# HumanCompatibleAI/imitation

Hardware: AMD Instinct MI355X
Metric: env-steps/sec (gen+disc round) GAIL HalfCheetah n_envs=1024 (higher is better)
Workload: dtype f32

## Files before the change

imitation_amd/csrc/policy.hip:

```cpp
#include "common.h"
#include "rn_common.h"
#include <algorithm>
#include <type_traits>
#include <cstring>

#include "../../include/imitation_hip.h"
#include "policy_common.h"

namespace {


template <int H>
struct Lds {
  static constexpr int XS = MAXD + 1, HS = H + 1, AS = MAXA + 1;
  static constexpr int x = 0;
  static constexpr int a1 = x + ROWS * XS;
  static constexpr int a2 = a1 + ROWS * HS;
  static constexpr int dz = a2 + ROWS * HS;
  static constexpr int out = dz + ROWS * HS;
  static constexpr int dout = out + ROWS * AS;
  static constexpr int aux = dout + ROWS * AS;
  static constexpr int total = aux + ROWS * AS + 64;
};

// ... 1443 lines not shown
            dst = b0 + cc * rows + r;
          }
        };
        tr(o.pW1, H, D); tr(o.pW2, H, H); tr(o.vW1, H, D); tr(o.vW2, H, H);
        Pt[dst] = pn;
      }
    }
  }
  if (next_batch > 0 && !stats_block) {
    __syncthreads();
    prepare_stats(d, obs, adv, next_idx, next_batch, T, n_envs, update_norm, nm, nv, ncount, w.advstat, lds);
  }
}

struct CLds {
  static constexpr int RS = 68;
  static constexpr int x = 0;
  static constexpr int a1 = x + MAXD * RS;
  static constexpr int a2 = a1 + 2 * 32 * RS;
  static constexpr int dz2 = a2 + 2 * 32 * RS;
  static constexpr int dz1 = dz2 + 2 * 32 * RS;
  static constexpr int dout = dz1 + 2 * 32 * RS;
  static constexpr int aux = dout + MAXA * RS;
  static constexpr int misc = aux + MAXA * RS;
  static constexpr int scratch = misc + 8 * RS;
  static constexpr int total = scratch + 64;
};


#ifndef IA_UPD_TSTR
#define IA_UPD_TSTR 36
#endif
constexpr int UPD_TSTR = IA_UPD_TSTR;
__host__ __device__ inline int upd_tbase(int off) { return (off * UPD_TSTR + 31) >> 5; }
__host__ __device__ inline int upd_pt4(int P4) { return (upd_tbase(P4) + 3) & ~3; }

template <bool SMALL>
__device__ __forceinline__ void chain_stage_rows(const ia_policy_desc& d, const float* __restrict__ nm,
                                                 const float* __restrict__ nv, const int i0, const int row_lim,
                                                 float* __restrict__ lds, const float* __restrict__ stg, const int tw,
                                                 const int q, const int lane) {
  using L = CLds;
  const int D = d.obs_dim;
  const int S1 = (D + 3) >> 2;
#ifndef IA_SMALL_STAGE_ASIDE
#define IA_SMALL_STAGE_ASIDE 1
#endif
  constexpr int QS = (SMALL && IA_SMALL_STAGE_ASIDE) ? 1 : 0;
  const bool idle = SMALL && q != QS;
  if (!idle) {
    const int rbase = SMALL ? 0 : q * 16;
    const int l128 = lane + 64 * tw;
    const int s1r = (65536 + S1 - 1) / S1;
    for (int g = l128; g < 16 * S1; g += 128) {
      const int r = (g * s1r) >> 16, k0 = (g - r * S1) * 4;
      const bool rok = (i0 + rbase + r) < row_lim;
      float raw[4], mu[4], vr[4];
      {
        const f32x4 rq = *reinterpret_cast<const f32x4*>(stg + UpdStage::x + (rbase * S1 + g) * 4);
        const f32x4 mq = *reinterpret_cast<const f32x4*>(nm + k0);
        const f32x4 vq = *reinterpret_cast<const f32x4*>(nv + k0);
#pragma unroll
        for (int j = 0; j < 4; ++j) {
          raw[j] = rq[j];
          mu[j] = mq[j];
          vr[j] = vq[j];
// ... 30 lines not shown
  const float* __restrict__ stg = stg_in + opaque_zero;
  float* __restrict__ slab = LOCAL ? stg_in + opaque_zero + UpdStage::x : slab_g;
  unsigned long long* __restrict__ slab64 = reinterpret_cast<unsigned long long*>(slab_g);
  auto put = [&](float* p, float v) {
    if constexpr (LOCAL) *p = v;
    else if (ll_xcd) ll_store_xcd(slab64 + (p - slab), v, ll_seq);
    else ll_store_agent(slab64 + (p - slab), v, ll_seq);
  };
  const int batch = rows.batch;
  constexpr int H = 32;
  using L = CLds;
#define IA_TS(slot) do { if (tstamp && i0_in == 0 && threadIdx.x == 0) tstamp[slot] = clock64(); } while (0)
  const int tid = threadIdx.x + opaque_zero, lane = tid & 63;
  const int wv = __builtin_amdgcn_readfirstlane(tid >> 6);
  const int tw = TSPLIT ? split_tw : (SMALL ? (wv & 1) : (wv >> 2)), q = SMALL ? (wv >> 1) : (wv & 3);
  const bool helper = TSPLIT && wv >= 4;
  const int li = lane & 15, lk = lane >> 4;
  const int D = d.obs_dim, A = d.act_dim;
  const PolOff o = pol_offsets(D, A, H, d.discrete);
  const int i0 = i0_in;
  const int aw = d.discrete ? 1 : A;
  const float invB = 1.f / (float)batch;
  const int S1 = (D + 3) >> 2;
  const int oW1 = tw ? o.vW1 : o.pW1, ob1 = tw ? o.vb1 : o.pb1, oW2 = tw ? o.vW2 : o.pW2, ob2 = tw ? o.vb2 : o.pb2;
  const float* __restrict__ sP = sP_in + opaque_zero;
  const float* __restrict__ sPt = sP + ((o.total + 3) & ~3);
  constexpr int TS_ = UPD_TSTR;
  const int tW1 = upd_tbase(oW1), tW2 = upd_tbase(oW2);
  IA_TS(0);

  const int lrow = q * 16 + (lane & 15);
  const bool valid = (i0 + lrow) < row_lim;
  float r_oldlp = 0.f, r_adv = 0.f, r_ret = 0.f, r_act[4] = {0.f, 0.f, 0.f, 0.f};
  constexpr bool HANDOVER = SMALL;
  if (helper) {
  } else if (tw == 0) {
    r_oldlp = stg[UpdStage::oldlp + lrow];
    if constexpr (!HANDOVER) r_adv = stg[UpdStage::adv + lrow];
#pragma unroll
    for (int j = 0; j < 4; ++j) r_act[j] = stg[UpdStage::act + lrow * aw + min(4 * (lane >> 4) + j, aw - 1)];
  } else {
    r_ret = stg[UpdStage::ret + lrow];
    if constexpr (HANDOVER) r_adv = stg[UpdStage::adv + lrow];
  }
  float* gconst = lds + L::scratch + 32;

  IA_TS(9);
  const bool idle = (SMALL && q > 0) || helper;
  if constexpr (!STAGED) chain_stage_rows<SMALL>(d, nm, nv, i0, row_lim, lds, stg, tw, q, lane);
  IA_TS(10);
  constexpr int KT1 = KS1 / 4;
  float fW1[KT1][2][4], fW2[2][2][4], fW2T[2][2][4], fHead[2][4], fHeadT[2][4], b1c[2][4], b2c[2][4], hb[4];
  const int head_base = tw == 0 ? o.aW + min(li, A - 1) * H : o.cW;
  float c_ivar[4] = {1.f, 1.f, 1.f, 1.f}, c_logsd[4] = {0.f, 0.f, 0.f, 0.f};
  if (!helper) {
#pragma unroll
  for (int kt = 0; kt < KT1; ++kt) {
    if (4 * kt < S1) {
#pragma unroll
      for (int t = 0; t < 2; ++t)
#pragma unroll
        for (int r = 0; r < 4; ++r) fW1[kt][t][r] = sPt[tW1 + min(16 * kt + 4 * lk + r, D - 1) * TS_ + 16 * t + li];
    } else {
#pragma unroll
      for (int t = 0; t < 2; ++t)
#pragma unroll
        for (int r = 0; r < 4; ++r) fW1[kt][t][r] = 0.f;
    }
  }
#pragma unroll
  for (int t = 0; t < 2; ++t)
#pragma unroll
    for (int r = 0; r < 4; ++r) b1c[t][r] = sP[ob1 + 16 * t + 4 * lk + r];
  float my_sd = sP[o.log_std + min(lane, A - 1)];
  __builtin_amdgcn_sched_barrier(0);
#pragma unroll
  for (int kt = 0; kt < KT1; ++kt)
#pragma unroll
    for (int t = 0; t < 2; ++t)
#pragma unroll
      for (int r = 0; r < 4; ++r) fW1[kt][t][r] = (16 * kt + 4 * lk + r < D) ? fW1[kt][t][r] : 0.f;
  if constexpr (HANDOVER) {
    if (tw != 0) {
      if (!idle) {
        float advn = r_adv;
        if (normalize_adv && batch > 1) advn = (advn - adv_mean) / (adv_std + 1e-8f);
        if (lk == 0) stg_in[opaque_zero + UpdStage::adv + lrow] = advn;
      }
      if (q == 0 && !d.discrete) {
        const float sd = expf(my_sd);
        const float my_ivar = lane < A ? 1.f / (sd * sd) : 1.f;
        const float my_logsd = lane < A ? logf(sd) : 0.f;
        if (lane < 16) {
          gconst[lane] = my_ivar;
          gconst[16 + lane] = my_logsd;
        }
      }
    }
  } else {
    float my_ivar = 1.f, my_logsd = 0.f;
    if (tw == 0 && !d.discrete) {
      const float sd = expf(my_sd);
      my_ivar = lane < A ? 1.f / (sd * sd) : 1.f;
      my_logsd = lane < A ? logf(sd) : 0.f;
    }
#pragma unroll
    for (int j = 0; j < 4; ++j) {
      c_ivar[j] = __shfl(my_ivar, 4 * lk + j, 64);
      c_logsd[j] = __shfl(my_logsd, 4 * lk + j, 64);
    }
  }
  }
  IA_TS(11);
  __syncthreads();
  IA_TS(1);

  float* a1t = lds + L::a1 + tw * 32 * L::RS;
  float* a2t = lds + L::a2 + tw * 32 * L::RS;
  float* dz2t = lds + L::dz2 + tw * 32 * L::RS;
  float* dz1t = lds + L::dz1 + tw * 32 * L::RS;
  const int trow = 4 * lk * L::RS + q * 16 + li;
  auto xchg16 = [](float v, float& a, float& b) {
    const auto p2 = __builtin_amdgcn_permlane16_swap(__float_as_uint(v), __float_as_uint(v), false, false);
    a = __uint_as_float(p2[0]);
    b = __uint_as_float(p2[1]);
  };
  auto xchg32 = [](float v, float& a, float& b) {
    const auto p2 = __builtin_amdgcn_permlane32_swap(__float_as_uint(v), __float_as_uint(v), false, false);
    a = __uint_as_float(p2[0]);
    b = __uint_as_float(p2[1]);
  };
  auto group_sum = [&](float v) {
    float a, b;
    xchg16(v, a, b);
    v = a + b;
    xchg32(v, a, b);
    return a + b;
  };
  auto group_max = [&](float v) {
    float a, b;
    xchg16(v, a, b);
    v = fmaxf(a, b);
    xchg32(v, a, b);
    return fmaxf(a, b);
  };
  if (!idle) {
  f32x4 a1[2], a2[2];
  {
    f32x4 acc[2][2] = {{{b1c[0][0], b1c[0][1], b1c[0][2], b1c[0][3]}, {0.f, 0.f, 0.f, 0.f}},
                       {{b1c[1][0], b1c[1][1], b1c[1][2], b1c[1][3]}, {0.f, 0.f, 0.f, 0.f}}};
    float xb[KT1][4];
#pragma unroll
    for (int kt = 0; kt < KT1; ++kt)
#pragma unroll
      for (int r = 0; r < 4; ++r) xb[kt][r] = lds[L::x + min(16 * kt + 4 * lk + r, MAXD - 1) * L::RS + q * 16 + li];
    if (HANDOVER && tw == 0) {
      r_adv = stg_in[opaque_zero + UpdStage::adv + lrow];
#pragma unroll
      for (int j = 0; j < 4; ++j) {
        c_ivar[j] = gconst[4 * lk + j];
        c_logsd[j] = gconst[16 + 4 * lk + j];
      }
    }
    __builtin_amdgcn_sched_barrier(0);
#pragma unroll
    for (int kt = 0; kt < KT1; ++kt)
      if (4 * kt < S1) {
#pragma unroll
        for (int r = 0; r < 4; ++r) {
          acc[0][kt & 1] = mfma16(fW1[kt][0][r], xb[kt][r], acc[0][kt & 1]);
          acc[1][kt & 1] = mfma16(fW1[kt][1][r], xb[kt][r], acc[1][kt & 1]);
        }
      }
#pragma unroll
    for (int kt = 0; kt < 2; ++kt)
#pragma unroll
      for (int r = 0; r < 4; ++r)
#pragma unroll
        for (int t = 0; t < 2; ++t) fW2[kt][t][r] = sPt[tW2 + (16 * kt + 4 * lk + r) * TS_ + 16 * t + li];
#pragma unroll
    for (int t = 0; t < 2; ++t)
#pragma unroll
      for (int r = 0; r < 4; ++r) b2c[t][r] = sP[ob2 + 16 * t + 4 * lk + r];
#pragma unroll
    for (int t = 0; t < 2; ++t)
#pragma unroll
      for (int r = 0; r < 4; ++r) {
        a1[t][r] = fast_tanh(acc[t][0][r] + acc[t][1][r]);
        a1t[trow + (16 * t + r) * L::RS] = a1[t][r];
// ... 71 lines not shown
          const float diff = r_act[j] - hout[j];
          logp += -(diff * diff) * (0.5f * c_ivar[j]) - c_logsd[j] - LOG_SQRT_2PI;
          entropy += 0.5f + LOG_SQRT_2PI + c_logsd[j];
        }
      logp = group_sum(logp);
      entropy = group_sum(entropy);
    } else {
      float mx = -3.0e38f, o_act = 0.f;
#pragma unroll
      for (int j = 0; j < 4; ++j)
        if (4 * lk + j < A) {
          mx = fmaxf(mx, hout[j]);
          o_act += (4 * lk + j == act_i) ? hout[j] : 0.f;
        }
      mx = group_max(mx);
      o_act = group_sum(o_act);
      float se = 0.f;
#pragma unroll
      for (int j = 0; j < 4; ++j)
        if (4 * lk + j < A) se += expf(hout[j] - mx);
      lse = mx + logf(group_sum(se));
      logp = o_act - lse;
#pragma unroll
      for (int j = 0; j < 4; ++j)
        if (4 * lk + j < A) {
          const float l = hout[j] - lse;
          entropy -= expf(l) * l;
        }
      entropy = group_sum(entropy);
    }
    IA_TS(13);
    float advn = r_adv;
    if constexpr (!HANDOVER)
      if (normalize_adv && batch > 1) advn = (advn - adv_mean) / (adv_std + 1e-8f);
    const float log_ratio = logp - r_oldlp;
    const float ratio = expf(log_ratio);
    const float lo = 1.f - clip, hi = 1.f + clip;
    const float pl1 = advn * ratio;
    const float pl2 = advn * fminf(fmaxf(ratio, lo), hi);
    const float g1 = pl1 < pl2 ? 1.f : (pl1 == pl2 ? 0.5f : 0.f);
    const float g2 = pl2 < pl1 ? 1.f : (pl1 == pl2 ? 0.5f : 0.f);
    const float inrange = (ratio >= lo && ratio <= hi) ? 1.f : 0.f;
    const float dlogp = valid ? -invB * advn * (g1 + g2 * inrange) * ratio : 0.f;
    IA_TS(14);
    float* doutrow = lds + L::dout + lrow;
    float* auxrow = lds + L::aux + lrow;
    if (!d.discrete) {
#pragma unroll
      for (int j = 0; j < 4; ++j)
        if (4 * lk + j < A) {
          const float diff = r_act[j] - hout[j];
          dout[j] = dlogp * diff * c_ivar[j];
          doutrow[(4 * lk + j) * L::RS] = dout[j];
          auxrow[(4 * lk + j) * L::RS] = valid ? dlogp * (diff * diff * c_ivar[j] - 1.f) - ent_coef * invB : 0.f;
        }
    } else {
#pragma unroll
      for (int j = 0; j < 4; ++j)
        if (4 * lk + j < A) {
          const float l = hout[j] - lse, p = expf(l);
          const float dH = -p * (l + entropy);
          float g = dlogp * ((4 * lk + j == act_i ? 1.f : 0.f) - p);
          g += valid ? -ent_coef * invB * dH : 0.f;
          dout[j] = g;
          doutrow[(4 * lk + j) * L::RS] = g;
        }
    }
// ... 2175 lines not shown
        stats[(long long)mb * 8 + kk] = sv;
        s_st[kk] = sv;
      }
      __syncthreads();
      if (tid == 0) {
        stats[(long long)mb * 8 + 5] = s_st[0] + ent_coef * s_st[2] + vf_coef * s_st[1];
        stats[(long long)mb * 8 + 6] = total_norm;
        stats[(long long)mb * 8 + 7] = coef;
      }
    }
    EP_TS(4);
  }
  tid = threadIdx.x;
#pragma unroll
  for (int j = 0; j < NPC; ++j) {
    const int i = bid * chunk + tid + j * NT;
    if (i < min(o.total, (bid + 1) * chunk)) {
      m[i] = m_[j];
      v[i] = v_[j];
      P[i] = p_[j];
      int dst = i;
      auto tr = [&](int b0, int rows_, int cols) {
        if (i >= b0 && i < b0 + rows_ * cols) {
          const int r = (i - b0) / cols, cc = (i - b0) % cols;
          dst = b0 + cc * rows_ + r;
        }
      };
      tr(o.pW1, H, D); tr(o.pW2, H, H); tr(o.vW1, H, D); tr(o.vW2, H, H);
      Pt[dst] = p_[j];
    }
  }
#undef EP_TS
}

template <int NPT, bool TIMING, int KS1, bool LOCAL, bool SHARD, bool SMALL, bool TSPLIT>
__device__ __forceinline__ void ppo_update_body(
    const ia_policy_desc& d, float* __restrict__ P, float* __restrict__ Pt, float* __restrict__ m, float* __restrict__ v,
    float* __restrict__ nm, float* __restrict__ nv, int32_t* __restrict__ ncount, int update_norm,
    const float* __restrict__ obs, const float* __restrict__ actions, const float* __restrict__ old_logp,
    const float* __restrict__ adv, const float* __restrict__ ret, const int64_t* __restrict__ perm, int T, int n_envs,
    int normalize_adv, float clip, float ent_coef, float vf_coef, float max_norm, float beta1, float beta2, float eps,
    float* __restrict__ ws, int nblk, int n_slices, float* __restrict__ stats, UpdSched sch, int xcd_pack,
    long long* __restrict__ tstamp ,
    ShardArgs sh) {
  constexpr int H = 32;
  using L = CLds;
  extern __shared__ float lds_raw[];
  float* lds = lds_raw + (((16u - (__builtin_amdgcn_groupstaticsize() & 15u)) & 15u) >> 2);
  __shared__ int s_ok, s_pub, s_fail, s_pubw[4];
  if (!TIMING) tstamp = nullptr;
  long long tacc[12] = {0, 0, 0, 0, 0, 0, 0, 0, 0, 0, 0, 0};
  long long tprev = 0;
#define UPD_TS(k) do { if (tstamp && tid == 0) { const long long tn = wall_clock64(); tacc[k] += tn - tprev; tprev = tn; } } while (0)
  if (xcd_pack && (blockIdx.x & 7)) return;
  const int vb = xcd_pack ? blockIdx.x >> 3 : blockIdx.x;
  static_assert(!TSPLIT || (!LOCAL && !SHARD && !SMALL), "one tower per workgroup: several gradient workgroups, one process");
  const int ngw = TSPLIT ? 2 * nblk : nblk;
  const int rb = TSPLIT ? vb >> 1 : vb;
  const int split_tw = TSPLIT ? (vb & 1) : 0;
  const int tid = threadIdx.x;
  const int D = d.obs_dim;
  const PolOff o = pol_offsets(D, d.act_dim, H, d.discrete);
  const UpdWs w = upd_ws(ws, nblk, o.total);
  unsigned* arrivals = w.ctrl + 64;
  unsigned* published = w.ctrl + 1;
  unsigned* sliced = w.ctrl + 16;
// ... 217 lines not shown
    const int jj = vb - ngw - 1;
    const int j = jj / NPH;
    if (j >= n_slices) return;
    for (int s = jj - j * NPH; s < n_steps; s += NPH) {
      const MbRows r = rows_of(s);
      const int r0 = j * UPD_SLICE;
      const int nr = min(UPD_SLICE, r.batch - r0);
      if (s >= UPD_RING) {
        if (tid == 0) s_ok = spin_until(published, (unsigned)(s - UPD_RING + 1), err);
        __syncthreads();
        if (!s_ok) return;
      }
      if (nr > 0) {
        float* pj = w.pring + ((long long)(s % UPD_RING) * UPD_SLICES_MAX + j) * UPD_PRS;
        prepare_stats_t<512>(d, r.obs, r.adv, r.idx + r0, nr, T, n_envs, update_norm, nullptr, nullptr, nullptr, nullptr,
                             lds, reinterpret_cast<int*>(lds + PREP_LDS_FLOATS), pj);
      }
      __syncthreads();
      if (tid == 0) {
        __threadfence();
        if (NPH == 1 || s == 0 || spin_until(sliced + j, (unsigned)s, err))
          __hip_atomic_store(sliced + j, (unsigned)(s + 1), __ATOMIC_RELAXED, __HIP_MEMORY_SCOPE_AGENT);
      }
    }
    return;
  }

  constexpr int PROWS = SMALL ? 16 : ROWS;
  float* sP = lds + L::total;
  float* sPt = sP + w.P4;
  float* stg = sPt + upd_pt4(w.P4);
  unsigned short* dstT = reinterpret_cast<unsigned short*>(stg + UpdStage::total(d.discrete ? 1 : d.act_dim));
  const int lane = tid & 63;
  float rm[NPT], rv[NPT];
#pragma unroll
  for (int k = 0; k < NPT; ++k) {
    const int i = tid + k * 512;
    rm[k] = rv[k] = 0.f;
    if (i < o.total) {
      const float pi_ = P[i];
      sP[i] = pi_;
      rm[k] = m[i];
      rv[k] = v[i];
      int dst = 0xffff;
      auto tr = [&](int base, int rows, int cols) {
        if (i >= base && i < base + rows * cols) {
          const int rr = (i - base) / cols, cc = (i - base) % cols;
          dst = upd_tbase(base) + cc * UPD_TSTR + rr;
        }
      };
      tr(o.pW1, H, D); tr(o.pW2, H, H); tr(o.vW1, H, D); tr(o.vW2, H, H);
      dstT[i] = (unsigned short)dst;
      if (dst != 0xffff) sPt[dst] = pi_;
    }
  }
  auto prefetch_resolve = [&](const MbRows& r) {
    if (tid >= 448) {
      int tz;
      asm volatile("s_mov_b32 %0, 0" : "=s"(tz));
      const unsigned Tq = (unsigned)(T + tz);
      const int i0 = row_lo + rb * ROWS;
      int src = 0;
      if (i0 + lane < row_lim(r)) {
        const long long flat = r.idx[i0 + lane];
        if (sch_total < (1ll << 31)) {
          const unsigned f = (unsigned)flat, env = f / Tq, t = f - env * Tq;
          src = (int)(t * (unsigned)n_envs + env);
        } else {
          src = (int)rollout_offset(flat, T, n_envs);
        }
      }
      reinterpret_cast<int*>(stg)[UpdStage::nxt + lane] = src;
    }
  };
  typedef __attribute__((address_space(3))) void* lds_void_p;
  typedef __attribute__((address_space(1))) const void* glb_void_p;
  const int wave = __builtin_amdgcn_readfirstlane(tid >> 6);
  auto prefetch_issue = [&](const MbRows& r, int zero) {
    const int* nxt = reinterpret_cast<const int*>(stg) + UpdStage::nxt;
    constexpr int SCW = 7;
    int src0 = 0;
    if (wave == SCW) src0 = nxt[lane];
    const int Q = (D + 3) >> 2;
    constexpr int NQT = (PROWS * (MAXD / 4) + 511) / 512;
    int qsrc[NQT], qoff[NQT];
// ... 31 lines not shown
      if (e0 < PROWS * Q)
        __builtin_amdgcn_global_load_lds((glb_void_p)(r.obs + (long long)qsrc[it] * D + qoff[it]),
                                         (lds_void_p)(stg + UpdStage::x + 4 * e0), 16, 0, 0);
    }
#pragma unroll
    for (int it = 0; it < NAT; ++it) {
      const int e0 = it * 512 + wave * 64;
      if (e0 < PROWS * aw_)
        __builtin_amdgcn_global_load_lds((glb_void_p)(r.actions + (long long)asrc[it] * aw_ + acol[it]),
                                         (lds_void_p)(stg + UpdStage::act + e0), 4, 0, 0);
    }
    if (wave == SCW) {
      __builtin_amdgcn_global_load_lds((glb_void_p)(r.old_logp + src0), (lds_void_p)(stg + UpdStage::oldlp), 4, 0, 0);
      __builtin_amdgcn_global_load_lds((glb_void_p)(r.adv + src0), (lds_void_p)(stg + UpdStage::adv), 4, 0, 0);
      __builtin_amdgcn_global_load_lds((glb_void_p)(r.ret + src0), (lds_void_p)(stg + UpdStage::ret), 4, 0, 0);
    }
  };
  auto prefetch_park = [&]() {
    if (wave == 0) stg[UpdStage::src + lane] = stg[UpdStage::nxt + lane];
    asm volatile("s_waitcnt vmcnt(0)" ::: "memory");
  };
  for (int e = tid; e < (SMALL ? L::total : MAXD * L::RS); e += 512) lds[L::x + e] = 0.f;
  int cur_e = sch_first / sch_nmb, cur_mb = sch_first - cur_e * sch_nmb;
  if (n_steps > 0) {
    prefetch_resolve(rows_at(cur_e, cur_mb));
    __syncthreads();
    prefetch_issue(rows_at(cur_e, cur_mb), 0);
    prefetch_park();
  }
  __syncthreads();

  bool have_ring = false;
  constexpr bool local = LOCAL;
  if (tstamp && tid == 0) tprev = wall_clock64();
  for (int s = 0; s < n_steps; ++s) {
    const MbRows r = rows_at(cur_e, cur_mb);
    const bool wrap = cur_mb + 1 == sch_nmb;
    const int nxt_e = wrap ? cur_e + 1 : cur_e, nxt_mb = wrap ? 0 : cur_mb + 1;
    cur_e = nxt_e;
    cur_mb = nxt_mb;
    const float* slot = w.ring + (s % UPD_RING) * UPD_RS;
    float adv_mean, adv_std;
    if (!have_ring) {
      if (tid == 0) {
        s_ok = spin_until(published, (unsigned)(s + 1), err);
        __threadfence();
      }
      __syncthreads();
      if (!s_ok) return;
      {
        int sz;
        asm volatile("s_mov_b32 %0, 0" : "=s"(sz));
        if (tid < 2 * MAXD + 8) stg[UpdStage::ring + tid] = *reinterpret_cast<const volatile float*>(slot + tid + sz);
      }
      __syncthreads();
      if constexpr (!LOCAL) {
        int zz;
        asm volatile("s_mov_b32 %0, 0" : "=s"(zz));
        const int wv_ = __builtin_amdgcn_readfirstlane((tid + zz) >> 6);
        chain_stage_rows<false>(d, stg + UpdStage::ring, stg + UpdStage::ring + MAXD, row_lo + rb * ROWS, row_lim(r), lds, stg,
                                wv_ >> 2, wv_ & 3, lane);
      }
    }
    slot = stg + UpdStage::ring;
    const int pub_early = (int)__hip_atomic_load(published, __ATOMIC_RELAXED, __HIP_MEMORY_SCOPE_AGENT);
    adv_mean = slot[2 * MAXD];
    adv_std = slot[2 * MAXD + 1];
    UPD_TS(0);
    const float step_size = w.tab[s], bc2_sqrt = w.tab[UPD_MAX_STEPS + s];
    if (s + 1 < n_steps) prefetch_resolve(rows_at(nxt_e, nxt_mb));
    const int P8 = w.P4 + 8;
    const unsigned lseq = lseq_base + (unsigned)s + 1u;
    const int xpar = SHARD ? (int)((sh.seq_base + (unsigned)s) & 1u) : 0;
    unsigned long long* slabs_s = w.slabs64 + (long long)(s & 1) * nblk * P8;
    float* stat_base = w.statpart + (s % UPD_SD) * nblk * 8;
    int oz;
    asm volatile("s_mov_b32 %0, 0" : "=s"(oz));
    mfma32_minibatch_chain<KS1, LOCAL, SMALL, !LOCAL, TSPLIT>(d, slot, slot + MAXD, adv_mean, adv_std, r, row_lo + rb * ROWS, row_lim(r),
                                       normalize_adv, clip, ent_coef, vf_coef,
                                       reinterpret_cast<float*>(slabs_s + (long long)rb * P8), stat_base + vb * 8, lds, sP,
                                       stg, oz, (tstamp && (!TSPLIT || vb == 0)) ? tstamp + 16 : nullptr, lseq, ll_xcd, split_tw);
    UPD_TS(1);
    UPD_TS(7);
    UPD_TS(8);
    float g[NPT];
    unsigned long long tail_w = 0ull;
    const bool want_tail = !LOCAL && vb == 0 && tid < 64 && stats;
    if (local) {
      int gz;
      asm volatile("s_mov_b32 %0, 0" : "=s"(gz));
#pragma unroll
      for (int k = 0; k < NPT; ++k) g[k] = stg[UpdStage::x + gz + min(tid + k * 512, o.total - 1)];
      if constexpr (SHARD) asm volatile("s_waitcnt vmcnt(0)" ::: "memory");
      if (tid == 0) {
        s_ok = 1;
        s_pub = pub_early;
        asm volatile("buffer_inv sc1" ::: "memory");
      }
      __syncthreads();
    }
    if (s + 1 < n_steps) {
      int pz;
      asm volatile("s_mov_b32 %0, 0" : "=s"(pz));
      prefetch_issue(rows_at(nxt_e, nxt_mb), pz);
    }
    if constexpr (!LOCAL) {
      if (s + 1 < n_steps && wave < 3) {
        if (pub_early >= s + 2) {
          const float* nslot = w.ring + ((s + 1) % UPD_RING) * UPD_RS;
          __builtin_amdgcn_global_load_lds((glb_void_p)(nslot + wave * MAXD + lane),
                                           (lds_void_p)(stg + UpdStage::ring + wave * MAXD), 4, 0, 0);
        }
        if (lane == 0) s_pubw[wave] = pub_early;
      }
    }
    UPD_TS(9);
    if constexpr (LOCAL) {
      UPD_TS(10);
      UPD_TS(11);
    } else {
      using u64 = unsigned long long;
      const int SL = (P8 + ngw - 1) / ngw;
      const unsigned rcpSL = 0xffffffffu / (unsigned)SL + 1u;
      float* red = lds + L::a1;
      auto valid_el = [&](int gi) { return gi < o.total || (gi >= w.P4 && gi < w.P4 + 5); };
      bool fail = false;
      const long long t0 = wall_clock64();
      const long long local_timeout = 200000000ll;
      u64* sums_s = w.sums64 + (long long)(s & 1) * P8;
      auto emit = [&](int gi, float part) {
        if constexpr (SHARD) {
          const unsigned xseq = sh.seq_base + (unsigned)s + 1u;
          for (int rr = 0; rr < sh.world; ++rr)
            ll_store_system(sh.peer_recv[rr] + (long long)(xpar * sh.world + (sh.loopback ? rr : sh.rank)) * P8 + gi, part, xseq);
        } else if (ll_xcd) {
          ll_store_xcd(sums_s + gi, part, lseq);
        } else {
          ll_store_agent(sums_s + gi, part, lseq);
        }
      };
      {
      {
        u64 t[NPT];
        int gi_[NPT];
        unsigned need = 0u;
        int ez;
        asm volatile("s_mov_b32 %0, 0" : "=s"(ez));
#pragma unroll
        for (int k = 0; k < NPT; ++k) {
          const int f = tid + ez + k * 512;
          const int j = (int)__umulhi((unsigned)f, rcpSL), e = f - j * SL;
          const int gi = vb * SL + e;
          gi_[k] = min(j, nblk - 1) * P8 + min(gi, P8 - 1);
          if (f < nblk * SL && valid_el(gi)) need |= 1u << k;
        }
        unsigned it = 0;
        for (;; ) {
#pragma unroll
          for (int k = 0; k < NPT; ++k)
            t[k] = __hip_atomic_load(slabs_s + gi_[k], __ATOMIC_RELAXED, __HIP_MEMORY_SCOPE_AGENT);
          __builtin_amdgcn_sched_barrier(0);
          bool ok = true;
#pragma unroll
          for (int k = 0; k < NPT; ++k) ok = ok && (!((need >> k) & 1u) || (unsigned)(t[k] >> 32) == lseq);
          if (ok) break;
          __builtin_amdgcn_s_sleep(1);
          if ((++it & 255u) == 0 &&
              (__hip_atomic_load(err, __ATOMIC_RELAXED, __HIP_MEMORY_SCOPE_AGENT) || wall_clock64() - t0 > local_timeout)) {
            fail = true;
            break;
          }
        }
        if (tstamp && tid == 0) tstamp[40] += it;
#pragma unroll
        for (int k = 0; k < NPT; ++k) {
          const int f = tid + k * 512;
          if (f < nblk * SL) red[f] = ((need >> k) & 1u) ? __uint_as_float((unsigned)t[k]) : 0.f;
        }
      }
      UPD_TS(10);
      if (fail) s_fail = 1;
      __syncthreads();
      if (s_fail) {
        if (tid == 0) __hip_atomic_store(err, 1u, __ATOMIC_RELAXED, __HIP_MEMORY_SCOPE_AGENT);
        return;
      }
      for (int e = tid; e < SL; e += 512) {
        const int gi = vb * SL + e;
        float part = 0.f;
        int j = 0;
        for (; j + 8 <= nblk; j += 8) {
          float tt[8];
#pragma unroll
          for (int u = 0; u < 8; ++u) tt[u] = red[(j + u) * SL + e];
          __builtin_amdgcn_sched_barrier(0);
#pragma unroll
          for (int u = 0; u < 8; ++u) part += tt[u];
        }
        for (; j < nblk; ++j) part += red[j * SL + e];
        if (valid_el(gi)) emit(gi, part);
      }
      }
      if constexpr (SHARD) {
        const unsigned xseq = sh.seq_base + (unsigned)s + 1u;
        const u64* rbase = sh.recv + (long long)(xpar * sh.world) * P8;
        for (int e = tid; e < SL; e += 512) {
          const int gi = vb * SL + e;
          if (!valid_el(gi)) continue;
          u64 t[SHARD_WORLD_MAX];
          for (unsigned it = 0;;) {
#pragma unroll
            for (int rr = 0; rr < SHARD_WORLD_MAX; ++rr)
              t[rr] = __hip_atomic_load(rbase + (long long)min(rr, sh.world - 1) * P8 + gi, __ATOMIC_RELAXED,
                                        __HIP_MEMORY_SCOPE_SYSTEM);
            __builtin_amdgcn_sched_barrier(0);
            bool ok = true;
#pragma unroll
            for (int rr = 0; rr < SHARD_WORLD_MAX; ++rr) ok = ok && (rr >= sh.world || (unsigned)(t[rr] >> 32) == xseq);
            if (ok) break;
            __builtin_amdgcn_s_sleep(1);
            if ((++it & 255u) == 0 && (__hip_atomic_load(err, __ATOMIC_RELAXED, __HIP_MEMORY_SCOPE_AGENT) ||
                                       wall_clock64() - t0 > sh.timeout_ticks)) {
              fail = true;
              break;
            }
          }
          if (fail) {
            __hip_atomic_store(err, 2u, __ATOMIC_RELAXED, __HIP_MEMORY_SCOPE_AGENT);
            break;
          }
          float part = 0.f;
#pragma unroll
          for (int rr = 0; rr < SHARD_WORLD_MAX; ++rr)
            if (rr < sh.world) part += __uint_as_float((unsigned)t[rr]);
          if (ll_xcd) ll_store_xcd(sums_s + gi, part, lseq);
          else ll_store_agent(sums_s + gi, part, lseq);
        }
      }
      UPD_TS(11);
      const bool stage_ahead = (s + 1 < n_steps) && min(min(s_pubw[0], s_pubw[1]), s_pubw[2]) >= s + 2;
      if (stage_ahead) {
        const MbRows rn = rows_at(nxt_e, nxt_mb);
        int zz;
        asm volatile("s_mov_b32 %0, 0" : "=s"(zz));
        const int wv_ = __builtin_amdgcn_readfirstlane((tid + zz) >> 6);
        chain_stage_rows<false>(d, stg + UpdStage::ring, stg + UpdStage::ring + MAXD, row_lo + rb * ROWS, row_lim(rn), lds, stg,
                                wv_ >> 2, wv_ & 3, lane);
      }
      if (tid == 0) s_pub = stage_ahead ? s + 2 : 0;
      {
        u64 t[NPT];
        int ez;
        asm volatile("s_mov_b32 %0, 0" : "=s"(ez));
        unsigned it = 0;
        for (; !fail;) {
#pragma unroll
          for (int k = 0; k < NPT; ++k)
            t[k] = __hip_atomic_load(sums_s + min(tid + ez + k * 512, o.total - 1), __ATOMIC_RELAXED, __HIP_MEMORY_SCOPE_AGENT);
          tail_w = __hip_atomic_load(sums_s + w.P4 + ez + min(lane, 4), __ATOMIC_RELAXED, __HIP_MEMORY_SCOPE_AGENT);
          __builtin_amdgcn_sched_barrier(0);
          bool ok = !want_tail || (unsigned)(tail_w >> 32) == lseq;
#pragma unroll
          for (int k = 0; k < NPT; ++k) ok = ok && (unsigned)(t[k] >> 32) == lseq;
          if (ok) break;
          __builtin_amdgcn_s_sleep(1);
          if ((++it & 255u) == 0 &&
              (__hip_atomic_load(err, __ATOMIC_RELAXED, __HIP_MEMORY_SCOPE_AGENT) ||
               wall_clock64() - t0 > (SHARD ? sh.timeout_ticks : local_timeout))) {
            fail = true;
            break;
          }
        }
        if (tstamp && tid == 0) tstamp[41] += it;
#pragma unroll
        for (int k = 0; k < NPT; ++k) g[k] = __uint_as_float((unsigned)t[k]);
      }
      if (fail) s_fail = 1;
      if (vb == 0 && tid == 0) __hip_atomic_fetch_add(arrivals, 1u, __ATOMIC_RELAXED, __HIP_MEMORY_SCOPE_AGENT);
    }
    if constexpr (LOCAL) have_ring = (s + 1 < n_steps) && (s_pub >= s + 2);
    if (LOCAL && have_ring && wave < 3) {
      const float* nslot = w.ring + ((s + 1) % UPD_RING) * UPD_RS;
      __builtin_amdgcn_global_load_lds((glb_void_p)(nslot + wave * MAXD + lane),
                                       (lds_void_p)(stg + UpdStage::ring + wave * MAXD), 4, 0, 0);
    }
    UPD_TS(2);
// ... 48 lines not shown
          __builtin_amdgcn_sched_barrier(0);
          bool ok = true;
#pragma unroll
          for (int u = 0; u < SHARD_RB; ++u)
#pragma unroll
            for (int k = 0; k < NPT; ++k) ok = ok && (unsigned)(t[u][k] >> 32) == seq;
          if (ok) break;
          __builtin_amdgcn_s_sleep(1);
          if ((++it & 255u) == 0 &&
              (__hip_atomic_load(err, __ATOMIC_RELAXED, __HIP_MEMORY_SCOPE_AGENT) || wall_clock64() - t0 > sh.timeout_ticks)) {
            fail = true;
            break;
          }
        }
#pragma unroll
        for (int u = 0; u < SHARD_RB; ++u)
          if (r0 + u < W) {
#pragma unroll
            for (int k = 0; k < NPT; ++k) g[k] += __uint_as_float((unsigned)t[u][k]);
          }
      }
      if (fail) {
        __hip_atomic_store(err, 2u, __ATOMIC_RELAXED, __HIP_MEMORY_SCOPE_AGENT);
        s_ok = 0;
      }
      __syncthreads();
      if (!s_ok) return;
    }
#pragma unroll
    for (int k = 0; k < NPT; ++k) {
      if (tid + k * 512 >= o.total) g[k] = 0.f;
      sq += g[k] * g[k];
    }
    UPD_TS(4);
    int rz;
    asm volatile("s_mov_b32 %0, 0" : "=s"(rz));
    const float total_sq = block_sum512_dpp(sq, lds + L::scratch + rz, s & 1);
    if constexpr (!LOCAL) {
      if (s_fail) {
        if (tid == 0) __hip_atomic_store(err, SHARD ? 2u : 1u, __ATOMIC_RELAXED, __HIP_MEMORY_SCOPE_AGENT);
        return;
      }
      have_ring = (s + 1 < n_steps) && (s_pub >= s + 2);
    }
    UPD_TS(5);
    const float total_norm = sqrtf(total_sq);
    const float coef = fminf(max_norm / (total_norm + 1e-6f), 1.0f);
    if constexpr (!LOCAL) {
      if (vb == 0 && tid < 64 && stats) {
        const float st = __uint_as_float((unsigned)tail_w) * (1.f / (float)r.batch);
        const float st0 = __shfl(st, 0, 64), st1 = __shfl(st, 1, 64), st2 = __shfl(st, 2, 64);
        float* so = stats + (long long)(sch_first + s) * 8;
        if (lane < 5) so[lane] = st;
        if (lane == 5) so[5] = st0 + ent_coef * st2 + vf_coef * st1;
        if (lane == 6) so[6] = total_norm;
        if (lane == 7) so[7] = coef;
      }
    } else if constexpr (SHARD) {
      if (vb == 0 && tid < 64 && stats) {
        const unsigned long long* rbase = sh.recv + (long long)(xpar * sh.world) * (w.P4 + 8) + w.P4;
        const unsigned seq = sh.seq_base + (unsigned)s + 1u;
        const int rk = min(lane >> 3, sh.world - 1);
        unsigned long long tv;
        const long long t0 = wall_clock64();
        bool late = false;
        do {
          tv = __hip_atomic_load(rbase + rk * (w.P4 + 8) + (lane & 7), __ATOMIC_RELAXED, __HIP_MEMORY_SCOPE_SYSTEM);
          late = !__all((unsigned)(tv >> 32) == seq);
        } while (late && wall_clock64() - t0 < sh.timeout_ticks);
        if (late && lane == 0)
          __hip_atomic_store(err, 2u, __ATOMIC_RELAXED, __HIP_MEMORY_SCOPE_AGENT);
        float st = (lane >> 3) < sh.world ? __uint_as_float((unsigned)tv) : 0.f;
        {
          float acc = __shfl(st, lane & 7, 64);
          for (int r_ = 1; r_ < sh.world; ++r_) acc += __shfl(st, r_ * 8 + (lane & 7), 64);
          st = acc * (1.f / (float)r.batch);
        }
        const float st0 = __shfl(st, 0, 64), st1 = __shfl(st, 1, 64), st2 = __shfl(st, 2, 64);
        float* so = stats + (long long)(sch_first + s) * 8;
        if (lane < 5) so[lane] = st;
        if (lane == 5) so[5] = st0 + ent_coef * st2 + vf_coef * st1;
        if (lane == 6) so[6] = total_norm;
        if (lane == 7) so[7] = coef;
      }
    } else if (vb == 0) {
      if (s + 1 < n_steps) {
        if (tid == 0) {
          slab_store(w.normcoef + (s % UPD_SD) * 2, total_norm);
          slab_store(w.normcoef + (s % UPD_SD) * 2 + 1, coef);
        }
      } else {
        write_loss_stats(s, total_norm, coef);
      }
    }
    {
      float pv[NPT];
      int dt[NPT];
#pragma unroll
      for (int k = 0; k < NPT; ++k) {
        const int ic = min(tid + k * 512, o.total - 1);
        pv[k] = sP[ic];
        dt[k] = dstT[ic];
      }
      __builtin_amdgcn_sched_barrier(0);
      const float inv_bc2 = 1.f / bc2_sqrt;
#pragma unroll
      for (int k = 0; k < NPT; ++k) {
        const float gi = g[k] * coef;
        float mi = rm[k];
        mi = mi + (gi - mi) * (1.f - beta1);
        const float vi = rv[k] * beta2 + (1.f - beta2) * gi * gi;
        const float denom = __builtin_amdgcn_sqrtf(vi) * inv_bc2 + eps;
        float rd = __builtin_amdgcn_rcpf(denom);
        rd = __builtin_fmaf(rd, __builtin_fmaf(-denom, rd, 1.f), rd);
        pv[k] = pv[k] - step_size * (mi * rd);
        rm[k] = mi;
        rv[k] = vi;
      }
      __builtin_amdgcn_sched_barrier(0);
#pragma unroll
      for (int k = 0; k < NPT; ++k) {
        const int i = tid + k * 512;
        if (i < o.total) {
          sP[i] = pv[k];
          if (dt[k] != 0xffff) sPt[dt[k]] = pv[k];
        }
      }
    }
    UPD_TS(6);
    if (s + 1 < n_steps && (LOCAL || !have_ring)) prefetch_park();
    else if (local) asm volatile("s_waitcnt vmcnt(0)" ::: "memory");
    __syncthreads();
    if (local && tid == 0)
      __hip_atomic_fetch_add(arrivals + 16 * (vb & (UPD_ARR - 1)), 1u, __ATOMIC_RELAXED, __HIP_MEMORY_SCOPE_AGENT);
    UPD_TS(3);
  }
#undef UPD_TS
  if (tstamp && vb == 0 && tid == 0)
    for (int k = 0; k < 12; ++k) tstamp[k] += tacc[k];
  if (vb == 0 && tid == 0)
    __hip_atomic_store(w.ctrl + 9, lseq_base + (unsigned)n_steps, __ATOMIC_RELAXED, __HIP_MEMORY_SCOPE_AGENT);
  if (vb == 0) {
#pragma unroll
    for (int k = 0; k < NPT; ++k) {
      const int i = tid + k * 512;
      if (i < o.total) {
        const float pi_ = sP[i];
        P[i] = pi_;
        int dst = i;
        auto tr = [&](int base, int rows, int cols) {
          if (i >= base && i < base + rows * cols) {
            const int rr = (i - base) / cols, cc = (i - base) % cols;
            dst = base + cc * rows + rr;
          }
        };
        tr(o.pW1, H, D); tr(o.pW2, H, H); tr(o.vW1, H, D); tr(o.vW2, H, H);
        Pt[dst] = pi_;
        m[i] = rm[k];
        v[i] = rv[k];
      }
    }
  }
}

#define IA_UPD_KERNEL_PARAMS                                                                                              \
  ia_policy_desc d, float *__restrict__ P, float *__restrict__ Pt, float *__restrict__ m, float *__restrict__ v,         \
      float *__restrict__ nm, float *__restrict__ nv, int32_t *__restrict__ ncount, int update_norm,                     \
      const float *__restrict__ obs, const float *__restrict__ actions, const float *__restrict__ old_logp,              \
      const float *__restrict__ adv, const float *__restrict__ ret, const int64_t *__restrict__ perm, int T, int n_envs, \
      int normalize_adv, float clip, float ent_coef, float vf_coef, float max_norm, float beta1, float beta2, float eps, \
      float *__restrict__ ws, int nblk, int n_slices, float *__restrict__ stats, UpdSched sch, int xcd_pack,             \
      long long *__restrict__ tstamp, ShardArgs sh
#define IA_UPD_KERNEL_ARGS                                                                                               \
  d, P, Pt, m, v, nm, nv, ncount, update_norm, obs, actions, old_logp, adv, ret, perm, T, n_envs, normalize_adv, clip,    \
      ent_coef, vf_coef, max_norm, beta1, beta2, eps, ws, nblk, n_slices, stats, sch, xcd_pack, tstamp, sh
// ... 898 lines not shown
```

Baseline: 4.903 million.

## Split Adam update so helper waves defer layer-2 and head updates into next step

When the tower-split path is active, the Adam moment state is partitioned. All waves update the first-layer weights right after the gradient reduction. Helper waves hold the layer-2 and head moments and apply their update at the start of the next step, reading the gradient from an LDS image. Helper waves also take over advantage normalization and the log-std constants from the main waves, which shortens the critical path before the sync. This adds extra LDS writes of the gradient, adds register pressure for the split moment arrays, and relies on deferred parameter writes staying consistent with their later readers.

```diff
diff --git a/imitation_amd/csrc/policy.hip b/imitation_amd/csrc/policy.hip
--- a/imitation_amd/csrc/policy.hip
+++ b/imitation_amd/csrc/policy.hip
@@ -1499,6 +1499,10 @@
 #define IA_UPD_TSTR 36
 #endif
 constexpr int UPD_TSTR = IA_UPD_TSTR;
+#ifndef IA_UPD_SPLIT_ADAM
+#define IA_UPD_SPLIT_ADAM 1
+#endif
+constexpr bool UPD_SPLIT_ADAM = IA_UPD_SPLIT_ADAM != 0;
 __host__ __device__ inline int upd_tbase(int off) { return (off * UPD_TSTR + 31) >> 5; }
 __host__ __device__ inline int upd_pt4(int P4) { return (upd_tbase(P4) + 3) & ~3; }
 
@@ -1595,8 +1599,16 @@
   const int lrow = q * 16 + (lane & 15);
   const bool valid = (i0 + lrow) < row_lim;
   float r_oldlp = 0.f, r_adv = 0.f, r_ret = 0.f, r_act[4] = {0.f, 0.f, 0.f, 0.f};
-  constexpr bool HANDOVER = SMALL;
+  constexpr bool HELP_OVER = TSPLIT && UPD_SPLIT_ADAM;
+  constexpr bool HANDOVER = SMALL || HELP_OVER;
+  float h_sd = 0.f;
   if (helper) {
+    if constexpr (HELP_OVER) {
+      if (tw == 0) {
+        r_adv = stg[UpdStage::adv + lrow];
+        h_sd = sP[d.discrete ? 0 : o.log_std + min(lane, A - 1)];
+      }
+    }
   } else if (tw == 0) {
     r_oldlp = stg[UpdStage::oldlp + lrow];
     if constexpr (!HANDOVER) r_adv = stg[UpdStage::adv + lrow];
@@ -1604,7 +1616,7 @@
     for (int j = 0; j < 4; ++j) r_act[j] = stg[UpdStage::act + lrow * aw + min(4 * (lane >> 4) + j, aw - 1)];
   } else {
     r_ret = stg[UpdStage::ret + lrow];
-    if constexpr (HANDOVER) r_adv = stg[UpdStage::adv + lrow];
+    if constexpr (SMALL) r_adv = stg[UpdStage::adv + lrow];
   }
   float* gconst = lds + L::scratch + 32;
 
@@ -1643,7 +1655,8 @@
     for (int t = 0; t < 2; ++t)
 #pragma unroll
       for (int r = 0; r < 4; ++r) fW1[kt][t][r] = (16 * kt + 4 * lk + r < D) ? fW1[kt][t][r] : 0.f;
-  if constexpr (HANDOVER) {
+  if constexpr (HELP_OVER) {
+  } else if constexpr (HANDOVER) {
     if (tw != 0) {
       if (!idle) {
         float advn = r_adv;
@@ -1673,6 +1686,24 @@
       c_logsd[j] = __shfl(my_logsd, 4 * lk + j, 64);
     }
   }
+  (void)my_sd;
+  }
+  if constexpr (HELP_OVER) {
+    if (helper && tw == 0) {
+      float advn = r_adv;
+      if (normalize_adv && batch > 1) advn = (advn - adv_mean) / (adv_std + 1e-8f);
+      if (lk == 0) stg_in[opaque_zero + UpdStage::adv + lrow] = advn;
+      if (q == 0 && !d.discrete) {
+        const float sd = expf(h_sd);
+        const float my_ivar = lane < A ? 1.f / (sd * sd) : 1.f;
+        const float my_logsd = lane < A ? logf(sd) : 0.f;
+        if (lane < 16) {
+          gconst[lane] = my_ivar;
+          gconst[16 + lane] = my_logsd;
+        }
+      }
+    }
+    if (tstamp && i0_in == 0 && threadIdx.x == 256) tstamp[16] = clock64();
   }
   IA_TS(11);
   __syncthreads();
@@ -4380,6 +4411,39 @@
   float* stg = sPt + upd_pt4(w.P4);
   unsigned short* dstT = reinterpret_cast<unsigned short*>(stg + UpdStage::total(d.discrete ? 1 : d.act_dim));
   const int lane = tid & 63;
+  constexpr bool SPLITA = TSPLIT && UPD_SPLIT_ADAM;
+  constexpr int N1 = KS1 == 8 ? 3 : 5;
+  constexpr int N2 = 7;
+  constexpr int NW2 = H * H + H;
+  const int l1_lo = split_tw ? o.vW1 : 0;
+  const int n1 = (split_tw ? o.vW2 : o.pW2) - l1_lo;
+  const int l2_lo = split_tw ? o.vW2 : o.pW2, head_lo = split_tw ? o.cW : o.aW;
+  const int n2 = NW2 + (split_tw ? o.total - o.cW : o.cW - o.aW);
+  const bool helper_wave = TSPLIT && __builtin_amdgcn_readfirstlane(tid >> 6) >= 4;
+  auto el2 = [&](int e) { return e < NW2 ? l2_lo + e : head_lo + (e - NW2); };
+  float* gimg = lds + L::a2;
+  constexpr int stat_wave = SPLITA ? 4 : 0;
+  float m1[N1], v1[N1], m2[N2], v2[N2];
+  if constexpr (SPLITA) {
+#pragma unroll
+    for (int j = 0; j < N1; ++j) {
+      const int e = tid + 512 * j;
+      m1[j] = v1[j] = 0.f;
+      if (e < n1) {
+        m1[j] = m[l1_lo + e];
+        v1[j] = v[l1_lo + e];
+      }
+    }
+#pragma unroll
+    for (int j = 0; j < N2; ++j) {
+      const int e = tid - 256 + 256 * j;
+      m2[j] = v2[j] = 0.f;
+      if (helper_wave && e < n2) {
+        m2[j] = m[el2(e)];
+        v2[j] = v[el2(e)];
+      }
+    }
+  }
   float rm[NPT], rv[NPT];
 #pragma unroll
   for (int k = 0; k < NPT; ++k) {
@@ -4388,8 +4452,10 @@
     if (i < o.total) {
       const float pi_ = P[i];
       sP[i] = pi_;
-      rm[k] = m[i];
-      rv[k] = v[i];
+      if constexpr (!SPLITA) {
+        rm[k] = m[i];
+        rv[k] = v[i];
+      }
       int dst = 0xffff;
       auto tr = [&](int base, int rows, int cols) {
         if (i >= base && i < base + rows * cols) {
@@ -4496,8 +4562,46 @@
 
   bool have_ring = false;
   constexpr bool local = LOCAL;
+  float p2_coef = 0.f, p2_step = 0.f, p2_inv = 0.f;
+  auto adam_list = [&](auto& mm, auto& vv, auto idx, int e0, int stride, int n, int ew0, float coef_, float step_, float inv_) {
+    constexpr int NJ = sizeof(mm) / sizeof(float);
+    float pv[NJ], gg[NJ];
+    int dt[NJ];
+#pragma unroll
+    for (int j = 0; j < NJ; ++j) {
+      const int ic = idx(min(e0 + stride * j, n - 1));
+      pv[j] = sP[ic];
+      dt[j] = dstT[ic];
+      gg[j] = gimg[ic];
+    }
+    __builtin_amdgcn_sched_barrier(0);
+#pragma unroll
+    for (int j = 0; j < NJ; ++j)
+      if (ew0 + stride * j < n) {
+        const float gi = gg[j] * coef_;
+        float mi = mm[j];
+        mi = mi + (gi - mi) * (1.f - beta1);
+        const float vi = vv[j] * beta2 + (1.f - beta2) * gi * gi;
+        const float denom = __builtin_amdgcn_sqrtf(vi) * inv_ + eps;
+        float rd = __builtin_amdgcn_rcpf(denom);
+        rd = __builtin_fmaf(rd, __builtin_fmaf(-denom, rd, 1.f), rd);
+        const float pn = pv[j] - step_ * (mi * rd);
+        if (e0 + stride * j < n) {
+          mm[j] = mi;
+          vv[j] = vi;
+          sP[idx(e0 + stride * j)] = pn;
+          if (dt[j] != 0xffff) sPt[dt[j]] = pn;
+        }
+      }
+  };
+  auto adam_part2 = [&]() {
+    if (helper_wave) adam_list(m2, v2, el2, tid - 256, 256, n2, (wave - 4) * 64, p2_coef, p2_step, p2_inv);
+    if (tstamp && vb == 0 && tid == 256) tstamp[33] = clock64();
+  };
   if (tstamp && tid == 0) tprev = wall_clock64();
   for (int s = 0; s < n_steps; ++s) {
+    if constexpr (SPLITA)
+      if (s > 0) adam_part2();
     const MbRows r = rows_at(cur_e, cur_mb);
     const bool wrap = cur_mb + 1 == sch_nmb;
     const int nxt_e = wrap ? cur_e + 1 : cur_e, nxt_mb = wrap ? 0 : cur_mb + 1;
@@ -4549,7 +4653,8 @@
     UPD_TS(8);
     float g[NPT];
     unsigned long long tail_w = 0ull;
-    const bool want_tail = !LOCAL && vb == 0 && tid < 64 && stats;
+    const bool stat_lanes = SPLITA ? wave == stat_wave : tid < 64;
+    const bool want_tail = !LOCAL && vb == 0 && stat_lanes && stats;
     if (local) {
       int gz;
       asm volatile("s_mov_b32 %0, 0" : "=s"(gz));
@@ -4830,6 +4935,10 @@
       if (tid + k * 512 >= o.total) g[k] = 0.f;
       sq += g[k] * g[k];
     }
+    if constexpr (SPLITA) {
+#pragma unroll
+      for (int k = 0; k < NPT; ++k) gimg[tid + k * 512] = g[k];
+    }
     UPD_TS(4);
     int rz;
     asm volatile("s_mov_b32 %0, 0" : "=s"(rz));
@@ -4845,7 +4954,7 @@
     const float total_norm = sqrtf(total_sq);
     const float coef = fminf(max_norm / (total_norm + 1e-6f), 1.0f);
     if constexpr (!LOCAL) {
-      if (vb == 0 && tid < 64 && stats) {
+      if (vb == 0 && stat_lanes && stats) {
         const float st = __uint_as_float((unsigned)tail_w) * (1.f / (float)r.batch);
         const float st0 = __shfl(st, 0, 64), st1 = __shfl(st, 1, 64), st2 = __shfl(st, 2, 64);
         float* so = stats + (long long)(sch_first + s) * 8;
@@ -4891,6 +5000,13 @@
         write_loss_stats(s, total_norm, coef);
       }
     }
+    if constexpr (SPLITA) {
+      const float inv_bc2 = 1.f / bc2_sqrt;
+      adam_list(m1, v1, [&](int e) { return l1_lo + e; }, tid, 512, n1, wave * 64, coef, step_size, inv_bc2);
+      p2_coef = coef;
+      p2_step = step_size;
+      p2_inv = inv_bc2;
+    } else
     {
       float pv[NPT];
       int dt[NPT];
@@ -4902,8 +5018,7 @@
       }
       __builtin_amdgcn_sched_barrier(0);
       const float inv_bc2 = 1.f / bc2_sqrt;
-#pragma unroll
-      for (int k = 0; k < NPT; ++k) {
+      auto adam_el = [&](int k) {
         const float gi = g[k] * coef;
         float mi = rm[k];
         mi = mi + (gi - mi) * (1.f - beta1);
@@ -4914,16 +5029,19 @@
         pv[k] = pv[k] - step_size * (mi * rd);
         rm[k] = mi;
         rv[k] = vi;
-      }
-      __builtin_amdgcn_sched_barrier(0);
-#pragma unroll
-      for (int k = 0; k < NPT; ++k) {
+      };
+      auto put_el = [&](int k) {
         const int i = tid + k * 512;
         if (i < o.total) {
           sP[i] = pv[k];
           if (dt[k] != 0xffff) sPt[dt[k]] = pv[k];
         }
-      }
+      };
+#pragma unroll
+      for (int k = 0; k < NPT; ++k) adam_el(k);
+      __builtin_amdgcn_sched_barrier(0);
+#pragma unroll
+      for (int k = 0; k < NPT; ++k) put_el(k);
     }
     UPD_TS(6);
     if (s + 1 < n_steps && (LOCAL || !have_ring)) prefetch_park();
@@ -4938,7 +5056,32 @@
     for (int k = 0; k < 12; ++k) tstamp[k] += tacc[k];
   if (vb == 0 && tid == 0)
     __hip_atomic_store(w.ctrl + 9, lseq_base + (unsigned)n_steps, __ATOMIC_RELAXED, __HIP_MEMORY_SCOPE_AGENT);
-  if (vb == 0) {
+  if constexpr (SPLITA) {
+    if (n_steps > 0) adam_part2();
+    if (rb == 0) {
+      auto wb = [&](int i, float mi, float vi) {
+        const float pi_ = sP[i];
+        P[i] = pi_;
+        int dst = i;
+        auto tr = [&](int base, int rows, int cols) {
+          if (i >= base && i < base + rows * cols) {
+            const int rr = (i - base) / cols, cc = (i - base) % cols;
+            dst = base + cc * rows + rr;
+          }
+        };
+        tr(o.pW1, H, D); tr(o.pW2, H, H); tr(o.vW1, H, D); tr(o.vW2, H, H);
+        Pt[dst] = pi_;
+        m[i] = mi;
+        v[i] = vi;
+      };
+#pragma unroll
+      for (int j = 0; j < N1; ++j)
+        if (tid + 512 * j < n1) wb(l1_lo + tid + 512 * j, m1[j], v1[j]);
+#pragma unroll
+      for (int j = 0; j < N2; ++j)
+        if (helper_wave && tid - 256 + 256 * j < n2) wb(el2(tid - 256 + 256 * j), m2[j], v2[j]);
+    }
+  } else if (vb == 0) {
 #pragma unroll
     for (int k = 0; k < NPT; ++k) {
       const int i = tid + k * 512;
```

Result: slower. 4.664 million (-4.9%).

## Offload update constants to helper, split hop-1 reduction, prefetch Adam params

Applied to the files above, without the earlier changes.

In the time-split PPO update, the helper wave group now normalizes advantages and computes the per-action inverse variance and log-std constants, handing them to the policy waves through LDS and staging memory. The first gradient-reduction hop is restructured so that only one of the two split groups owns the slab reduction, with a register-resident summation path for small block counts. Parameter values and packed transpose indices are also loaded before the spin-wait and kept in registers for the Adam step. The aim is to shorten the critical path and cut redundant global loads, at the cost of more register pressure and more complex synchronisation.

```diff
diff --git a/imitation_amd/csrc/policy.hip b/imitation_amd/csrc/policy.hip
--- a/imitation_amd/csrc/policy.hip
+++ b/imitation_amd/csrc/policy.hip
@@ -1596,10 +1596,16 @@
   const bool valid = (i0 + lrow) < row_lim;
   float r_oldlp = 0.f, r_adv = 0.f, r_ret = 0.f, r_act[4] = {0.f, 0.f, 0.f, 0.f};
   constexpr bool HANDOVER = SMALL;
+#ifndef IA_UPD_HELPER_CONSTS
+#define IA_UPD_HELPER_CONSTS 1
+#endif
+  const bool hand_t = TSPLIT && IA_UPD_HELPER_CONSTS && tw == 0;
   if (helper) {
+    if (hand_t) r_adv = stg[UpdStage::adv + lrow];
   } else if (tw == 0) {
     r_oldlp = stg[UpdStage::oldlp + lrow];
-    if constexpr (!HANDOVER) r_adv = stg[UpdStage::adv + lrow];
+    if constexpr (!HANDOVER)
+      if (!hand_t) r_adv = stg[UpdStage::adv + lrow];
 #pragma unroll
     for (int j = 0; j < 4; ++j) r_act[j] = stg[UpdStage::act + lrow * aw + min(4 * (lane >> 4) + j, aw - 1)];
   } else {
@@ -1661,6 +1667,7 @@
       }
     }
   } else {
+    if (!hand_t) {
     float my_ivar = 1.f, my_logsd = 0.f;
     if (tw == 0 && !d.discrete) {
       const float sd = expf(my_sd);
@@ -1672,7 +1679,21 @@
       c_ivar[j] = __shfl(my_ivar, 4 * lk + j, 64);
       c_logsd[j] = __shfl(my_logsd, 4 * lk + j, 64);
     }
-  }
+    }
+  }
+  } else if (hand_t) {
+    float advn = r_adv;
+    if (normalize_adv && batch > 1) advn = (advn - adv_mean) / (adv_std + 1e-8f);
+    if (lk == 0) stg_in[opaque_zero + UpdStage::adv + lrow] = advn;
+    if (q == 0 && !d.discrete) {
+      const float sd = expf(sP[o.log_std + min(lane, A - 1)]);
+      const float my_ivar = lane < A ? 1.f / (sd * sd) : 1.f;
+      const float my_logsd = lane < A ? logf(sd) : 0.f;
+      if (lane < 16) {
+        gconst[lane] = my_ivar;
+        gconst[16 + lane] = my_logsd;
+      }
+    }
   }
   IA_TS(11);
   __syncthreads();
@@ -1717,7 +1738,7 @@
     for (int kt = 0; kt < KT1; ++kt)
 #pragma unroll
       for (int r = 0; r < 4; ++r) xb[kt][r] = lds[L::x + min(16 * kt + 4 * lk + r, MAXD - 1) * L::RS + q * 16 + li];
-    if (HANDOVER && tw == 0) {
+    if ((HANDOVER && tw == 0) || hand_t) {
       r_adv = stg_in[opaque_zero + UpdStage::adv + lrow];
 #pragma unroll
       for (int j = 0; j < 4; ++j) {
@@ -1855,7 +1876,7 @@
     IA_TS(13);
     float advn = r_adv;
     if constexpr (!HANDOVER)
-      if (normalize_adv && batch > 1) advn = (advn - adv_mean) / (adv_std + 1e-8f);
+      if (!hand_t && normalize_adv && batch > 1) advn = (advn - adv_mean) / (adv_std + 1e-8f);
     const float log_ratio = logp - r_oldlp;
     const float ratio = expf(log_ratio);
     const float lo = 1.f - clip, hi = 1.f + clip;
@@ -4097,6 +4118,9 @@
   }
 #undef EP_TS
 }
+
+template <int N>
+struct UpdIntC { static constexpr int value = N; };
 
 template <int NPT, bool TIMING, int KS1, bool LOCAL, bool SHARD, bool SMALL, bool TSPLIT>
 __device__ __forceinline__ void ppo_update_body(
@@ -4381,6 +4405,13 @@
   unsigned short* dstT = reinterpret_cast<unsigned short*>(stg + UpdStage::total(d.discrete ? 1 : d.act_dim));
   const int lane = tid & 63;
   float rm[NPT], rv[NPT];
+#ifndef IA_UPD_ADAM_EARLY
+#define IA_UPD_ADAM_EARLY 1
+#endif
+  constexpr bool ADAM_EARLY = TSPLIT && IA_UPD_ADAM_EARLY;
+  unsigned dtp[(NPT + 1) / 2];
+#pragma unroll
+  for (int k = 0; k < (NPT + 1) / 2; ++k) dtp[k] = 0xffffffffu;
 #pragma unroll
   for (int k = 0; k < NPT; ++k) {
     const int i = tid + k * 512;
@@ -4399,6 +4430,7 @@
       };
       tr(o.pW1, H, D); tr(o.pW2, H, H); tr(o.vW1, H, D); tr(o.vW2, H, H);
       dstT[i] = (unsigned short)dst;
+      if constexpr (ADAM_EARLY) dtp[k >> 1] = (k & 1) ? ((dtp[k >> 1] & 0xffffu) | ((unsigned)dst << 16)) : ((dtp[k >> 1] & 0xffff0000u) | (unsigned)dst);
       if (dst != 0xffff) sPt[dst] = pi_;
     }
   }
@@ -4548,6 +4580,7 @@
     UPD_TS(7);
     UPD_TS(8);
     float g[NPT];
+    float pv_e[ADAM_EARLY ? NPT : 1];
     unsigned long long tail_w = 0ull;
     const bool want_tail = !LOCAL && vb == 0 && tid < 64 && stats;
     if (local) {
@@ -4584,7 +4617,17 @@
       UPD_TS(11);
     } else {
       using u64 = unsigned long long;
-      const int SL = (P8 + ngw - 1) / ngw;
+#ifndef IA_UPD_HOP1_VALUE
+#define IA_UPD_HOP1_VALUE 1
+#endif
+#ifndef IA_UPD_REGSUM
+#define IA_UPD_REGSUM 1
+#endif
+      constexpr bool OWN_V = TSPLIT && IA_UPD_HOP1_VALUE;
+      const int nown = OWN_V ? nblk : ngw;
+      const int own = OWN_V ? rb : vb;
+      const bool owner = !OWN_V || split_tw != 0;
+      const int SL = (P8 + nown - 1) / nown;
       const unsigned rcpSL = 0xffffffffu / (unsigned)SL + 1u;
       float* red = lds + L::a1;
       auto valid_el = [&](int gi) { return gi < o.total || (gi >= w.P4 && gi < w.P4 + 5); };
@@ -4603,7 +4646,72 @@
           ll_store_agent(sums_s + gi, part, lseq);
         }
       };
-      {
+      bool hop1_done = false;
+      if constexpr (TSPLIT) {
+        const int EL = (SL + 511) >> 9;
+        if (!owner) {
+          UPD_TS(10);
+          asm volatile("s_waitcnt vmcnt(0)" ::: "memory");
+          __syncthreads();
+          hop1_done = true;
+        } else if (IA_UPD_REGSUM && nblk <= 16 && (nblk <= 2 ? 2 : nblk <= 4 ? 4 : nblk <= 8 ? 8 : 16) * EL <= 16) {
+          auto regsum = [&](auto gc) {
+            constexpr int G = decltype(gc)::value, NE = 16 / G;
+            u64 t[NE][G];
+            int ez;
+            asm volatile("s_mov_b32 %0, 0" : "=s"(ez));
+            const int e0 = own * SL + tid + ez;
+            bool nd[NE];
+#pragma unroll
+            for (int i = 0; i < NE; ++i) nd[i] = tid + 512 * i < SL && valid_el(own * SL + tid + 512 * i);
+            unsigned it = 0;
+            for (;;) {
+#pragma unroll
+              for (int i = 0; i < NE; ++i)
+#pragma unroll
+                for (int j = 0; j < G; ++j)
+                  t[i][j] = __hip_atomic_load(slabs_s + min(j, nblk - 1) * P8 + min(e0 + 512 * i, P8 - 1), __ATOMIC_RELAXED,
+                                              __HIP_MEMORY_SCOPE_AGENT);
+              __builtin_amdgcn_sched_barrier(0);
+              bool ok = true;
+#pragma unroll
+              for (int i = 0; i < NE; ++i)
+#pragma unroll
+                for (int j = 0; j < G; ++j) ok = ok && (!nd[i] || (unsigned)(t[i][j] >> 32) == lseq);
+              if (ok) break;
+              __builtin_amdgcn_s_sleep(1);
+              if ((++it & 255u) == 0 &&
+                  (__hip_atomic_load(err, __ATOMIC_RELAXED, __HIP_MEMORY_SCOPE_AGENT) || wall_clock64() - t0 > local_timeout)) {
+                fail = true;
+                break;
+              }
+            }
+            if (tstamp && tid == 0) tstamp[40] += it;
+            UPD_TS(10);
+            if (!fail) {
+#pragma unroll
+              for (int i = 0; i < NE; ++i) {
+                float part = 0.f;
+#pragma unroll
+                for (int j = 0; j < G; ++j) part += j < nblk ? __uint_as_float((unsigned)t[i][j]) : 0.f;
+                if (nd[i]) emit(e0 + 512 * i, part);
+              }
+            }
+          };
+          if (nblk <= 2) regsum(UpdIntC<2>{});
+          else if (nblk <= 4) regsum(UpdIntC<4>{});
+          else if (nblk <= 8) regsum(UpdIntC<8>{});
+          else regsum(UpdIntC<16>{});
+          if (fail) s_fail = 1;
+          __syncthreads();
+          if (s_fail) {
+            if (tid == 0) __hip_atomic_store(err, 1u, __ATOMIC_RELAXED, __HIP_MEMORY_SCOPE_AGENT);
+            return;
+          }
+          hop1_done = true;
+        }
+      }
+      if (!hop1_done) {
       {
         u64 t[NPT];
         int gi_[NPT];
@@ -4614,7 +4722,7 @@
         for (int k = 0; k < NPT; ++k) {
           const int f = tid + ez + k * 512;
           const int j = (int)__umulhi((unsigned)f, rcpSL), e = f - j * SL;
-          const int gi = vb * SL + e;
+          const int gi = own * SL + e;
           gi_[k] = min(j, nblk - 1) * P8 + min(gi, P8 - 1);
           if (f < nblk * SL && valid_el(gi)) need |= 1u << k;
         }
@@ -4650,7 +4758,7 @@
         return;
       }
       for (int e = tid; e < SL; e += 512) {
-        const int gi = vb * SL + e;
+        const int gi = own * SL + e;
         float part = 0.f;
         int j = 0;
         for (; j + 8 <= nblk; j += 8) {
@@ -4716,6 +4824,10 @@
         u64 t[NPT];
         int ez;
         asm volatile("s_mov_b32 %0, 0" : "=s"(ez));
+        if constexpr (ADAM_EARLY) {
+#pragma unroll
+          for (int k = 0; k < NPT; ++k) pv_e[k] = sP[min(tid + ez + k * 512, o.total - 1)];
+        }
         unsigned it = 0;
         for (; !fail;) {
 #pragma unroll
@@ -4897,8 +5009,13 @@
 #pragma unroll
       for (int k = 0; k < NPT; ++k) {
         const int ic = min(tid + k * 512, o.total - 1);
-        pv[k] = sP[ic];
-        dt[k] = dstT[ic];
+        if constexpr (ADAM_EARLY) {
+          pv[k] = pv_e[k];
+          dt[k] = (int)((dtp[k >> 1] >> (16 * (k & 1))) & 0xffffu);
+        } else {
+          pv[k] = sP[ic];
+          dt[k] = dstT[ic];
+        }
       }
       __builtin_amdgcn_sched_barrier(0);
       const float inv_bc2 = 1.f / bc2_sqrt;
@@ -4936,6 +5053,10 @@
 #undef UPD_TS
   if (tstamp && vb == 0 && tid == 0)
     for (int k = 0; k < 12; ++k) tstamp[k] += tacc[k];
+  if (TSPLIT && tstamp && vb == 1 && tid == 0) {
+    tstamp[32] += tacc[10];
+    tstamp[33] += tacc[11];
+  }
   if (vb == 0 && tid == 0)
     __hip_atomic_store(w.ctrl + 9, lseq_base + (unsigned)n_steps, __ATOMIC_RELAXED, __HIP_MEMORY_SCOPE_AGENT);
   if (vb == 0) {
```

Result: slower. 5.094 million before, 3.929 million after (-22.9%).
